# vccheng2001/DeepVCP-Pointcloud-Registration

Hardware: AMD Instinct MI355X
Metric: pairs/sec (full DeepVCP forward) at N=16384, K=64; rot/trans error vs ref (higher is better)
Workload: dtype f32

## Files before the change

### deepvcp-pointcloud-registration_amd/csrc/ball_query.hip

```cpp
#include "common.h"
#include "morton.h"


namespace dvcp {

template <typename T>
struct alignas(16) PointSS {
  T x, y, z, ss;
};

constexpr int kBqThreads = 256;

template <typename T>
__global__ __launch_bounds__(kBqThreads) void ball_query_kernel(
    PointsView<T> pts, int N, PointsView<T> ctr, int S, T r2, int nsample,
    int32_t* __restrict__ count, int32_t* __restrict__ list, int64_t* __restrict__ padded) {
  constexpr int TILE = (sizeof(T) == 4) ? 1024 : 512;
  __shared__ PointSS<T> tile[TILE];
  const int b = blockIdx.y;
  const int s = blockIdx.x * kBqThreads + threadIdx.x;
  const bool live = s < S;
  T cx = 0, cy = 0, cz = 0;
  if (live) {
    cx = ctr.at(b, 0, s);
    cy = ctr.at(b, 1, s);
    cz = ctr.at(b, 2, s);
  }
  const T ssc = sumsq3(cx, cy, cz);
  const int64_t row = (static_cast<int64_t>(b) * S + s) * nsample;
  int32_t* my_list = list ? list + row : nullptr;
  int64_t* my_pad = padded ? padded + row : nullptr;
  int cnt = 0;
  int first = N;
  bool done = !live;

  for (int t0 = 0; t0 < N; t0 += TILE) {
    const int nt = min(TILE, N - t0);
    __syncthreads();
    for (int j = threadIdx.x; j < nt; j += kBqThreads) {
      const T x = pts.at(b, 0, t0 + j), y = pts.at(b, 1, t0 + j), z = pts.at(b, 2, t0 + j);
      tile[j] = PointSS<T>{x, y, z, sumsq3(x, y, z)};
    }
    __syncthreads();
    if (!done) {
      for (int j = 0; j < nt; ++j) {
        const PointSS<T> p = tile[j];
        const T d2 = expansion_d2(dot3_blas(cx, cy, cz, p.x, p.y, p.z), ssc, p.ss);
        if (!(d2 > r2)) {
          const int n = t0 + j;
          if (cnt == 0) first = n;
          if (my_list) my_list[cnt] = n;
          if (my_pad) my_pad[cnt] = n;
          if (++cnt == nsample) {
            done = true;
            break;
          }
        }
      }
    }
    if (__syncthreads_and(done)) break;
  }
  if (!live) return;
  if (count) count[static_cast<int64_t>(b) * S + s] = cnt;
  if (my_list && cnt == 0) my_list[0] = 0;
  if (my_pad)
    for (int j = cnt; j < nsample; ++j) my_pad[j] = first;
}


__host__ __device__ constexpr int bq_padded_n(int N) { return (N + 15) & ~15; }

constexpr int kBqTile = 64;
#ifndef DVCP_BQ_ABL
#define DVCP_BQ_ABL 0
#endif
constexpr int kBqMaxTiles = 1024;
constexpr int kBqSmallTiles = 256;
constexpr int kBqCap = 256;

struct BqLayout {
  float4* packed;
  float4* sorted;
  float4* tbox;
  int32_t* cperm;
};

inline int64_t bq_align(int64_t x) { return (x + 255) & ~int64_t(255); }

inline BqLayout bq_layout(void* ws, int B, int N, int S) {
  const int64_t T = ceil_div(N, kBqTile);
  char* p = static_cast<char*>(ws);
  BqLayout L;
  L.packed = reinterpret_cast<float4*>(p);
  p += bq_align(16 * int64_t(B) * bq_padded_n(N));
  L.sorted = reinterpret_cast<float4*>(p);
  p += bq_align(16 * int64_t(B) * T * kBqTile);
  L.tbox = reinterpret_cast<float4*>(p);
  p += bq_align(32 * int64_t(B) * T);
  L.cperm = reinterpret_cast<int32_t*>(p);
  return L;
}

inline int64_t bq_workspace_bytes(int B, int N, int S) {
  const int64_t T = ceil_div(N, kBqTile);
  return bq_align(16 * int64_t(B) * bq_padded_n(N)) + bq_align(16 * int64_t(B) * T * kBqTile) +
         bq_align(32 * int64_t(B) * T) + bq_align(4 * int64_t(B) * S);
}

__global__ void bq_pack_kernel(PointsView<float> pts, int N, float4* __restrict__ packed) {
  const int b = blockIdx.y;
  const int n = blockIdx.x * blockDim.x + threadIdx.x;
  const int np = bq_padded_n(N);
  if (n >= np) return;
  float4 v = make_float4(0.f, 0.f, 0.f, 0.f);
  if (n < N) {
    const float x = pts.at(b, 0, n), y = pts.at(b, 1, n), z = pts.at(b, 2, n);
    v = make_float4(x, y, z, sumsq3(x, y, z));
  }
  packed[static_cast<int64_t>(b) * np + n] = v;
}

__global__ __launch_bounds__(kBuildThreads) void bq_build_kernel(PointsView<float> pts, int N, PointsView<float> ctr,
                                                                 int S, BqLayout L, int tiled) {
  __shared__ uint32_t bins[kSortBins];
  __shared__ uint32_t boxk[kBqMaxTiles][6];
  __shared__ uint32_t wsum[16];
  __shared__ float red[2][3][16];
  const int b = blockIdx.y, tid = threadIdx.x;
  auto get_ctr = [&](int i, float (&v)[3]) {
#pragma unroll
    for (int a = 0; a < 3; ++a) v[a] = ctr.at(b, a, i);
  };
  float lo[3], hi[3];
  if (blockIdx.x == 1) {
    block_bbox(S, get_ctr, lo, hi, red);
    int32_t* cp = L.cperm + static_cast<int64_t>(b) * S;
    morton_sort(
        S, get_ctr, [&](int pos, int i, const float (&)[3]) { cp[pos] = i; }, lo, hi, bins, wsum);
    return;
  }
  const int np = bq_padded_n(N);
  float4* pk = L.packed + static_cast<int64_t>(b) * np;
  for (int i = tid; i < np; i += kBuildThreads) {
    float4 v = make_float4(0.f, 0.f, 0.f, 0.f);
    if (i < N) {
      const float x = pts.at(b, 0, i), y = pts.at(b, 1, i), z = pts.at(b, 2, i);
      v = make_float4(x, y, z, sumsq3(x, y, z));
    }
    pk[i] = v;
  }
  if (!tiled) return;
  const int T = (N + kBqTile - 1) / kBqTile;
  float4* so = L.sorted + static_cast<int64_t>(b) * T * kBqTile;
  for (int i = tid; i < T * 6; i += kBuildThreads) boxk[i / 6][i % 6] = (i % 6) < 3 ? 0xFFFFFFFFu : 0u;
  auto get_pt = [&](int i, float (&v)[3]) {
#pragma unroll
    for (int a = 0; a < 3; ++a) v[a] = pts.at(b, a, i);
  };
  block_bbox(N, get_pt, lo, hi, red);
  morton_sort(
      N, get_pt,
      [&](int pos, int i, const float (&v)[3]) {
        so[pos] = make_float4(v[0], v[1], v[2], __int_as_float(i));
        const int t = pos / kBqTile;
        const bool fin = __builtin_isfinite(v[0]) && __builtin_isfinite(v[1]) && __builtin_isfinite(v[2]);
#pragma unroll
        for (int a = 0; a < 3; ++a) {
          atomicMin(&boxk[t][a], float_order(fin ? v[a] : -__builtin_huge_valf()));
          atomicMax(&boxk[t][3 + a], float_order(fin ? v[a] : __builtin_huge_valf()));
        }
      },
      lo, hi, bins, wsum);
  for (int pos = N + tid; pos < T * kBqTile; pos += kBuildThreads)
    so[pos] = make_float4(__builtin_nanf(""), __builtin_nanf(""), __builtin_nanf(""), __int_as_float(0x7FFFFFFF));
  for (int t = tid; t < T; t += kBuildThreads) {
    float4* tb = L.tbox + (static_cast<int64_t>(b) * T + t) * 2;
    tb[0] = make_float4(float_unorder(boxk[t][0]), float_unorder(boxk[t][1]), float_unorder(boxk[t][2]), 0.f);
    tb[1] = make_float4(float_unorder(boxk[t][3]), float_unorder(boxk[t][4]), float_unorder(boxk[t][5]), 0.f);
  }
}

__global__ __launch_bounds__(256) void bq_wave_kernel(const float4* __restrict__ packed, int N, PointsView<float> ctr,
                                                      int S, float r2, int nsample, int32_t* __restrict__ count,
                                                      int32_t* __restrict__ list, int64_t* __restrict__ padded) {
  const int b = blockIdx.y;
  const int s = blockIdx.x * 256 + threadIdx.x;
  if ((blockIdx.x * 256 + (threadIdx.x & ~63)) >= S) return;
  const bool live = s < S;
  float cx = 0.f, cy = 0.f, cz = 0.f;
  if (live) {
    cx = ctr.at(b, 0, s);
    cy = ctr.at(b, 1, s);
    cz = ctr.at(b, 2, s);
  }
  const float ssc = sumsq3(cx, cy, cz);
  const int64_t row = (static_cast<int64_t>(b) * S + s) * nsample;
  int cnt = live ? 0 : nsample;
  int first = N;
  const const_float* P = (const const_float*)uniform_ptr(packed + static_cast<int64_t>(b) * bq_padded_n(N));
  for (int n0 = 0; n0 < N; n0 += 16) {
    float c[64];
#pragma unroll
    for (int u = 0; u < 64; ++u) c[u] = P[4 * n0 + u];
#pragma unroll
    for (int j = 0; j < 16; ++j) {
      const int n = n0 + j;
      const float d2 = expansion_d2(dot3_blas(cx, cy, cz, c[4 * j], c[4 * j + 1], c[4 * j + 2]), ssc, c[4 * j + 3]);
      if ((n < N) & !(d2 > r2) & (cnt < nsample)) {
        first = cnt == 0 ? n : first;
        if (list) list[row + cnt] = n;
        if (padded) padded[row + cnt] = n;
        ++cnt;
      }
    }
    if (__ballot(cnt < nsample) == 0) break;
  }
  if (!live) return;
  if (count) count[static_cast<int64_t>(b) * S + s] = cnt;
  if (list && cnt == 0) list[row] = 0;
  if (padded)
    for (int j = cnt; j < nsample; ++j) padded[row + j] = first;
}

__device__ __forceinline__ float wave_fmin(float v) {
  for (int off = 32; off > 0; off >>= 1) v = fminf(v, __shfl_xor(v, off, kWave));
  return v;
}
__device__ __forceinline__ float wave_fmax(float v) {
  for (int off = 32; off > 0; off >>= 1) v = fmaxf(v, __shfl_xor(v, off, kWave));
  return v;
}

__device__ __forceinline__ float bq_prune_thr(float r2, float ssc_max, float ssp_max) {
  return (r2 + 0x1p-20f * (ssc_max + ssp_max)) * (1.0f + 0x1p-19f);
}

__device__ __forceinline__ float box_ss_max(float lx, float ly, float lz, float hx, float hy, float hz) {
  const float ax = fmaxf(fabsf(lx), fabsf(hx)), ay = fmaxf(fabsf(ly), fabsf(hy)), az = fmaxf(fabsf(lz), fabsf(hz));
  return ((ax * ax + ay * ay) + az * az) * (1.0f + 0x1p-20f);
}

__device__ __forceinline__ float bq_gap(float lo, float hi, float v_lo, float v_hi) {
  return fmaxf(fmaxf(v_lo - hi, lo - v_hi), 0.0f);
}

template <int MAXT>
__global__ __launch_bounds__(256) void bq_tiled_kernel(BqLayout L, int N, PointsView<float> ctr, int S, float r2,
                                                       int nsample, int32_t* __restrict__ count,
                                                       int32_t* __restrict__ list, int64_t* __restrict__ padded,
                                                       int xcd) {
  __shared__ uint32_t bm[4][MAXT * 2];
  __shared__ float4 cpt[4][kBqCap];
  __shared__ int32_t cid[4][kBqCap];
  int b = blockIdx.y, bx = blockIdx.x;
  if (xcd) {
    const int lin = static_cast<int>(blockIdx.y * gridDim.x + blockIdx.x);
    const int slot = lin >> 3;
    b = (lin & 7) + 8 * (slot / static_cast<int>(gridDim.x));
    bx = slot % static_cast<int>(gridDim.x);
  }
  const int wave = threadIdx.x >> 6, lane = threadIdx.x & 63;
  const int q0 = (bx * 4 + wave) * 64;
  if (q0 >= S) return;
  const int T = (N + kBqTile - 1) / kBqTile;
  const int NW = (N + 31) >> 5;
  const int np = bq_padded_n(N);
  const bool live = q0 + lane < S;
  const int s = live ? L.cperm[static_cast<int64_t>(b) * S + q0 + lane] : 0;
  float cx = 0.f, cy = 0.f, cz = 0.f;
  if (live) {
    cx = ctr.at(b, 0, s);
    cy = ctr.at(b, 1, s);
    cz = ctr.at(b, 2, s);
  }
  const float ssc = sumsq3(cx, cy, cz);
  const bool fin = __builtin_isfinite(cx) && __builtin_isfinite(cy) && __builtin_isfinite(cz);
  const float inf = __builtin_huge_valf();
  int cut1 = -1, cut2 = -1, cut3 = -1;
  if (__ballot(live && !fin) == 0) {
    const float rr2 = 2.0f * sqrtf(r2);
    const bool bl = live;
    auto box_vol = [&](const float (&lo)[3], const float (&hi)[3]) {
      return !(hi[0] >= lo[0]) ? 0.0f : ((hi[0] - lo[0] + rr2) * (hi[1] - lo[1] + rr2)) * (hi[2] - lo[2] + rr2);
    };
    auto best_cut = [&](int a, int e) -> int {
      const bool in = bl && lane >= a && lane < e;
      const float c3[3] = {cx, cy, cz};
      float plo[3], phi[3], slo[3], shi[3];
#pragma unroll
      for (int d = 0; d < 3; ++d) {
        plo[d] = slo[d] = in ? c3[d] : inf;
        phi[d] = shi[d] = in ? c3[d] : -inf;
      }
#pragma unroll
      for (int off = 1; off < 64; off <<= 1) {
#pragma unroll
        for (int d = 0; d < 3; ++d) {
          const float ul = __shfl_up(plo[d], off, kWave), uh = __shfl_up(phi[d], off, kWave);
          const float dl = __shfl_down(slo[d], off, kWave), dh = __shfl_down(shi[d], off, kWave);
          if (lane >= off) {
            plo[d] = fminf(plo[d], ul);
            phi[d] = fmaxf(phi[d], uh);
          }
          if (lane + off < 64) {
            slo[d] = fminf(slo[d], dl);
            shi[d] = fmaxf(shi[d], dh);
          }
        }
      }
      const float vp = box_vol(plo, phi);
      const float vs = box_vol(slo, shi);
      const float vprev = __shfl_up(vp, 1, kWave);
      const float whole = __shfl(vp, 63, kWave);
      const float cost = (lane > a && lane < e) ? vprev + vs : inf;
      float m = cost;
      for (int off = 32; off > 0; off >>= 1) m = fminf(m, __shfl_xor(m, off, kWave));
      if (!(m < 0.7f * whole)) return -1;
      return static_cast<int>(__builtin_ctzll(__ballot(cost == m)));
    };
    cut1 = best_cut(0, 64);
    if (cut1 > 0) {
      cut2 = best_cut(0, cut1);
      cut3 = best_cut(cut1, 64);
    }
  }
  const int ngroups = 1 + (cut1 >= 0) + (cut2 >= 0) + (cut3 >= 0);
  const int gid = (cut2 >= 0 && lane >= cut2) + (cut1 >= 0 && lane >= cut1) + (cut3 >= 0 && lane >= cut3);
  uint32_t* mybm = bm[wave];
  const float4* tb = L.tbox + static_cast<int64_t>(b) * T * 2;
  const float4* so = L.sorted + static_cast<int64_t>(b) * T * kBqTile;
  const float4* pk = L.packed + static_cast<int64_t>(b) * np;
  const int64_t row = (static_cast<int64_t>(b) * S + s) * nsample;
  int cnt = live ? 0 : nsample;
  int first = N;
  float4* mypt = cpt[wave];
  int32_t* myid = cid[wave];
  for (int g = 0; g < ngroups; ++g) {
    const bool act = live && gid == g;
    if (__ballot(act) == 0) continue;
    const float wlx = wave_fmin(act ? (fin ? cx : -inf) : inf), whx = wave_fmax(act ? (fin ? cx : inf) : -inf);
    const float wly = wave_fmin(act ? (fin ? cy : -inf) : inf), why = wave_fmax(act ? (fin ? cy : inf) : -inf);
    const float wlz = wave_fmin(act ? (fin ? cz : -inf) : inf), whz = wave_fmax(act ? (fin ? cz : inf) : -inf);
    const float ssc_max = wave_fmax(act && fin ? ssc : 0.0f);

    __builtin_amdgcn_fence(__ATOMIC_ACQ_REL, "wavefront");
    __builtin_amdgcn_wave_barrier();
    for (int i = lane; i < NW; i += 64) mybm[i] = 0u;
    __builtin_amdgcn_fence(__ATOMIC_RELEASE, "wavefront");
    __builtin_amdgcn_wave_barrier();
    for (int t0 = 0; t0 < T; t0 += 64) {
      const int t = t0 + lane;
      bool cand = false;
      if (t < T) {
        const float4 lo = tb[2 * t], hi = tb[2 * t + 1];
        const float gx = bq_gap(lo.x, hi.x, wlx, whx), gy = bq_gap(lo.y, hi.y, wly, why), gz = bq_gap(lo.z, hi.z, wlz, whz);
        const float lb2 = (gx * gx + gy * gy) + gz * gz;
        cand = !(lb2 > bq_prune_thr(r2, ssc_max, box_ss_max(lo.x, lo.y, lo.z, hi.x, hi.y, hi.z)));
      }
      uint64_t mask = __ballot(cand);
      while (mask) {
        int tt[4];
#pragma unroll
        for (int u = 0; u < 4; ++u) {
          tt[u] = mask ? t0 + __builtin_ctzll(mask) : -1;
          mask &= mask - 1;
        }
        float4 q[4];
#pragma unroll
        for (int u = 0; u < 4; ++u) q[u] = so[max(tt[u], 0) * kBqTile + lane];
#pragma unroll
        for (int u = 0; u < 4; ++u) {
          const int idx = __float_as_int(q[u].w);
          const float gx = bq_gap(q[u].x, q[u].x, wlx, whx), gy = bq_gap(q[u].y, q[u].y, wly, why),
                      gz = bq_gap(q[u].z, q[u].z, wlz, whz);
          const float lb2 = (gx * gx + gy * gy) + gz * gz;
          const float ssp = ((q[u].x * q[u].x + q[u].y * q[u].y) + q[u].z * q[u].z) * (1.0f + 0x1p-20f);
          if (tt[u] >= 0 && idx < N && !(lb2 > bq_prune_thr(r2, ssc_max, ssp)))
            atomicOr(&mybm[idx >> 5], 1u << (idx & 31));
        }
      }
    }
    __builtin_amdgcn_fence(__ATOMIC_ACQ_REL, "wavefront");
    __builtin_amdgcn_wave_barrier();

    for (int c0 = 0; c0 < NW; c0 += 64) {
      const uint32_t word = (c0 + lane < NW) ? mybm[c0 + lane] : 0u;
      const int pc = __builtin_popcount(word);
      int incl = pc;
#pragma unroll
      for (int off = 1; off < 64; off <<= 1) {
        const int u = __shfl_up(incl, off, kWave);
        if (lane >= off) incl += u;
      }
      const int total = __shfl(incl, 63, kWave);
      const int excl = incl - pc;
      for (int base = 0; base < total; base += kBqCap) {
        int p = excl;
        uint32_t wd = word;
        while (wd && p < base + kBqCap) {
          const int bit = __builtin_ctz(wd);
          wd &= wd - 1;
          if (p >= base) myid[p - base] = (c0 + lane) * 32 + bit;
          ++p;
        }
        __builtin_amdgcn_fence(__ATOMIC_ACQ_REL, "wavefront");
        __builtin_amdgcn_wave_barrier();
        const int nc = min(kBqCap, total - base);
#pragma unroll
        for (int u = 0; u < kBqCap / 64; ++u) {
          const int j = u * 64 + lane;
          if (j < nc) mypt[j] = pk[myid[j]];
        }
        __builtin_amdgcn_fence(__ATOMIC_ACQ_REL, "wavefront");
        __builtin_amdgcn_wave_barrier();
        for (int j0 = 0; j0 < nc; j0 += 64) {
          const int je = min(nc, j0 + 64);
          for (int j1 = j0; j1 < je; j1 += 8) {
            float4 q[8];
#pragma unroll
            for (int u = 0; u < 8; ++u) q[u] = mypt[j1 + u];
#pragma unroll
            for (int u = 0; u < 8; ++u) {
              const float d2 = expansion_d2(dot3_blas(cx, cy, cz, q[u].x, q[u].y, q[u].z), ssc, q[u].w);
              if (act & (j1 + u < je) & !(d2 > r2) & (cnt < nsample)) {
                const int n = myid[j1 + u];
                first = cnt == 0 ? n : first;
#if DVCP_BQ_ABL != 1
                if (list) list[row + cnt] = n;
#endif
                if (padded) padded[row + cnt] = n;
                ++cnt;
              }
            }
          }
          if (__ballot(act && cnt < nsample) == 0) goto group_done;
        }
        __builtin_amdgcn_fence(__ATOMIC_ACQ_REL, "wavefront");
        __builtin_amdgcn_wave_barrier();
      }
    }
  group_done:;
  }
  if (!live) return;
  if (count) count[static_cast<int64_t>(b) * S + s] = cnt;
  if (list && cnt == 0) list[row] = 0;
  if (padded)
    for (int j = cnt; j < nsample; ++j) padded[row + j] = first;
}

template <typename T>
__global__ void square_distance_kernel(PointsView<T> src, int S, PointsView<T> dst, int N, T* __restrict__ out) {
  const int b = blockIdx.z;
  const int s = blockIdx.y;
  const int n = blockIdx.x * blockDim.x + threadIdx.x;
  if (n >= N) return;
  const T sx = src.at(b, 0, s), sy = src.at(b, 1, s), sz = src.at(b, 2, s);
  const T dx = dst.at(b, 0, n), dy = dst.at(b, 1, n), dz = dst.at(b, 2, n);
  out[(static_cast<int64_t>(b) * S + s) * N + n] =
      expansion_d2(dot3_blas(sx, sy, sz, dx, dy, dz), sumsq3(sx, sy, sz), sumsq3(dx, dy, dz));
}

template <typename T>
static int launch_bq(const void* xyz, int64_t sb, int64_t sc, int64_t sn, int N, const void* c, int64_t cb,
                     int64_t cc, int64_t cn, int S, int B, double radius, int nsample, int32_t* count,
                     int32_t* list, int64_t* padded, void* workspace, hipStream_t st) {
  PointsView<T> pv{static_cast<const T*>(xyz), sb, sc, sn};
  PointsView<T> cv{static_cast<const T*>(c), cb, cc, cn};
  const T r2 = static_cast<T>(radius * radius);
  if constexpr (sizeof(T) == 4) {
    if (workspace) {
      const BqLayout L = bq_layout(workspace, B, N, S);
      const int tiled = N <= kBqMaxTiles * kBqTile;
      hipLaunchKernelGGL(bq_build_kernel, dim3(tiled ? 2 : 1, B), dim3(kBuildThreads), 0, st, pv, N, cv, S, L, tiled);
      if (int e = launch_status("dvcp_ball_query(build)")) return e;
      if (tiled)
        hipLaunchKernelGGL(N <= kBqSmallTiles * kBqTile ? bq_tiled_kernel<kBqSmallTiles> : bq_tiled_kernel<kBqMaxTiles>,
                           dim3(ceil_div(S, 256), B), dim3(256), 0, st, L, N, cv, S, r2, nsample, count, list, padded,
                           B % 8 == 0 ? 1 : 0);
      else
        hipLaunchKernelGGL(bq_wave_kernel, dim3(ceil_div(S, 256), B), dim3(256), 0, st, L.packed, N, cv, S, r2,
                           nsample, count, list, padded);
      return launch_status("dvcp_ball_query");
    }
  }
  dim3 grid(ceil_div(S, kBqThreads), B);
  hipLaunchKernelGGL((ball_query_kernel<T>), grid, dim3(kBqThreads), 0, st, pv, N, cv, S, r2, nsample, count,
                     list, padded);
  return launch_status("dvcp_ball_query");
}

}

extern "C" int dvcp_ball_query_ws(int dtype, const void* xyz, int64_t sb, int64_t sc, int64_t sn, int N,
                                  const void* ctr, int64_t cb, int64_t cc, int64_t cn, int S, int B,
                                  double radius, int nsample, int32_t* count, int32_t* list,
                                  int64_t* padded, void* workspace, void* stream) {
  DVCP_REQUIRE(xyz && ctr, "dvcp_ball_query: null pointer");
  DVCP_REQUIRE(N >= 0 && S >= 0 && B >= 0 && nsample > 0, "dvcp_ball_query: bad sizes");
  if (B == 0 || S == 0) return DVCP_OK;
  DVCP_REQUIRE(B <= 65535, "dvcp_ball_query: B too large");
  hipStream_t st = static_cast<hipStream_t>(stream);
  if (dtype == DVCP_F32)
    return dvcp::launch_bq<float>(xyz, sb, sc, sn, N, ctr, cb, cc, cn, S, B, radius, nsample, count, list,
                                  padded, workspace, st);
  if (dtype == DVCP_F64)
    return dvcp::launch_bq<double>(xyz, sb, sc, sn, N, ctr, cb, cc, cn, S, B, radius, nsample, count, list,
                                   padded, nullptr, st);
  dvcp::set_error("dvcp_ball_query: bad dtype %d", dtype);
  return DVCP_EINVAL;
}

extern "C" int64_t dvcp_ball_query_workspace_bytes(int B, int N, int S) {
  if (B < 0 || N < 0 || S < 0) return -1;
  return dvcp::bq_workspace_bytes(B, N, S);
}

extern "C" int dvcp_ball_query(int dtype, const void* xyz, int64_t sb, int64_t sc, int64_t sn, int N,
                               const void* ctr, int64_t cb, int64_t cc, int64_t cn, int S, int B,
                               double radius, int nsample, int32_t* count, int32_t* list,
                               int64_t* padded, void* stream) {
  return dvcp_ball_query_ws(dtype, xyz, sb, sc, sn, N, ctr, cb, cc, cn, S, B, radius, nsample, count, list, padded,
                            nullptr, stream);
}

extern "C" int dvcp_square_distance(int dtype, const void* src, int64_t sb, int64_t sc, int64_t sn, int S,
                                    const void* dst, int64_t db, int64_t dc, int64_t dn, int N, int B,
                                    void* out, void* stream) {
  DVCP_REQUIRE(src && dst && out, "dvcp_square_distance: null pointer");
  if (B == 0 || S == 0 || N == 0) return DVCP_OK;
  DVCP_REQUIRE(S <= 65535 && B <= 65535, "dvcp_square_distance: S/B too large");
  hipStream_t st = static_cast<hipStream_t>(stream);
  dim3 grid(dvcp::ceil_div(N, 256), S, B);
  if (dtype == DVCP_F32) {
    hipLaunchKernelGGL((dvcp::square_distance_kernel<float>), grid, dim3(256), 0, st,
                       dvcp::PointsView<float>{static_cast<const float*>(src), sb, sc, sn}, S,
                       dvcp::PointsView<float>{static_cast<const float*>(dst), db, dc, dn}, N,
                       static_cast<float*>(out));
  } else if (dtype == DVCP_F64) {
    hipLaunchKernelGGL((dvcp::square_distance_kernel<double>), grid, dim3(256), 0, st,
                       dvcp::PointsView<double>{static_cast<const double*>(src), sb, sc, sn}, S,
                       dvcp::PointsView<double>{static_cast<const double*>(dst), db, dc, dn}, N,
                       static_cast<double*>(out));
  } else {
    dvcp::set_error("dvcp_square_distance: bad dtype %d", dtype);
    return DVCP_EINVAL;
  }
  return dvcp::launch_status("dvcp_square_distance");
}
```

Before: 2531.

## Assign four lanes per query center in tiled ball query kernel

Restructures the tiled ball-query kernel so each wavefront handles 16 centers with 4 lanes per center. Candidates are split across the quad and hits are compacted in order with a ballot-based prefix. The candidate-bitmap compaction now walks contiguous per-lane word ranges instead of strided words. Group splitting drops from up to four groups to a single cut, candidate ids are stored as uint16, and launch bounds gain an occupancy hint. The aim is more parallelism per query and less serial hit scanning, at the cost of four times as many blocks, repeated tile culling per wave, and uint16 ids that limit indexable N.

```diff
diff --git a/deepvcp-pointcloud-registration_amd/csrc/ball_query.hip b/deepvcp-pointcloud-registration_amd/csrc/ball_query.hip
--- a/deepvcp-pointcloud-registration_amd/csrc/ball_query.hip
+++ b/deepvcp-pointcloud-registration_amd/csrc/ball_query.hip
@@ -71,12 +71,11 @@
 __host__ __device__ constexpr int bq_padded_n(int N) { return (N + 15) & ~15; }
 
 constexpr int kBqTile = 64;
-#ifndef DVCP_BQ_ABL
-#define DVCP_BQ_ABL 0
-#endif
 constexpr int kBqMaxTiles = 1024;
 constexpr int kBqSmallTiles = 256;
 constexpr int kBqCap = 256;
+constexpr int kBqQuad = 4;
+constexpr int kBqWaveCtr = kWave / kBqQuad;
 
 struct BqLayout {
   float4* packed;
@@ -230,6 +229,9 @@
   for (int off = 32; off > 0; off >>= 1) v = fmaxf(v, __shfl_xor(v, off, kWave));
   return v;
 }
+__device__ __forceinline__ float wave_uniform(float v) {
+  return __int_as_float(__builtin_amdgcn_readfirstlane(__float_as_int(v)));
+}
 
 __device__ __forceinline__ float bq_prune_thr(float r2, float ssc_max, float ssp_max) {
   return (r2 + 0x1p-20f * (ssc_max + ssp_max)) * (1.0f + 0x1p-19f);
@@ -245,13 +247,13 @@
 }
 
 template <int MAXT>
-__global__ __launch_bounds__(256) void bq_tiled_kernel(BqLayout L, int N, PointsView<float> ctr, int S, float r2,
-                                                       int nsample, int32_t* __restrict__ count,
-                                                       int32_t* __restrict__ list, int64_t* __restrict__ padded,
-                                                       int xcd) {
-  __shared__ uint32_t bm[4][MAXT * 2];
+__global__ __launch_bounds__(256, MAXT == kBqSmallTiles ? 6 : 3) void bq_tiled_kernel(
+    BqLayout L, int N, PointsView<float> ctr, int S, float r2, int nsample, int32_t* __restrict__ count,
+    int32_t* __restrict__ list, int64_t* __restrict__ padded, int xcd) {
+  constexpr int WPL = MAXT * 2 / kWave;
+  __shared__ alignas(16) uint32_t bm[4][MAXT * 2];
   __shared__ float4 cpt[4][kBqCap];
-  __shared__ int32_t cid[4][kBqCap];
+  __shared__ uint16_t cid[4][kBqCap];
   int b = blockIdx.y, bx = blockIdx.x;
   if (xcd) {
     const int lin = static_cast<int>(blockIdx.y * gridDim.x + blockIdx.x);
@@ -260,13 +262,13 @@
     bx = slot % static_cast<int>(gridDim.x);
   }
   const int wave = threadIdx.x >> 6, lane = threadIdx.x & 63;
-  const int q0 = (bx * 4 + wave) * 64;
+  const int ctrl = lane / kBqQuad, ql = lane % kBqQuad;
+  const int q0 = (bx * 4 + wave) * kBqWaveCtr;
   if (q0 >= S) return;
   const int T = (N + kBqTile - 1) / kBqTile;
-  const int NW = (N + 31) >> 5;
   const int np = bq_padded_n(N);
-  const bool live = q0 + lane < S;
-  const int s = live ? L.cperm[static_cast<int64_t>(b) * S + q0 + lane] : 0;
+  const bool live = q0 + ctrl < S;
+  const int s = live ? L.cperm[static_cast<int64_t>(b) * S + q0 + ctrl] : 0;
   float cx = 0.f, cy = 0.f, cz = 0.f;
   if (live) {
     cx = ctr.at(b, 0, s);
@@ -276,56 +278,57 @@
   const float ssc = sumsq3(cx, cy, cz);
   const bool fin = __builtin_isfinite(cx) && __builtin_isfinite(cy) && __builtin_isfinite(cz);
   const float inf = __builtin_huge_valf();
-  int cut1 = -1, cut2 = -1, cut3 = -1;
+  int cut = -1;
   if (__ballot(live && !fin) == 0) {
     const float rr2 = 2.0f * sqrtf(r2);
-    const bool bl = live;
     auto box_vol = [&](const float (&lo)[3], const float (&hi)[3]) {
       return !(hi[0] >= lo[0]) ? 0.0f : ((hi[0] - lo[0] + rr2) * (hi[1] - lo[1] + rr2)) * (hi[2] - lo[2] + rr2);
     };
-    auto best_cut = [&](int a, int e) -> int {
-      const bool in = bl && lane >= a && lane < e;
-      const float c3[3] = {cx, cy, cz};
-      float plo[3], phi[3], slo[3], shi[3];
+    const float c3[3] = {cx, cy, cz};
+    float lo[3], hi[3];
+#pragma unroll
+    for (int d = 0; d < 3; ++d) {
+      lo[d] = live ? c3[d] : inf;
+      hi[d] = live ? c3[d] : -inf;
+    }
+#pragma unroll
+    for (int off = kBqQuad; off < kWave; off <<= 1) {
 #pragma unroll
       for (int d = 0; d < 3; ++d) {
-        plo[d] = slo[d] = in ? c3[d] : inf;
-        phi[d] = shi[d] = in ? c3[d] : -inf;
-      }
-#pragma unroll
-      for (int off = 1; off < 64; off <<= 1) {
-#pragma unroll
-        for (int d = 0; d < 3; ++d) {
-          const float ul = __shfl_up(plo[d], off, kWave), uh = __shfl_up(phi[d], off, kWave);
-          const float dl = __shfl_down(slo[d], off, kWave), dh = __shfl_down(shi[d], off, kWave);
-          if (lane >= off) {
-            plo[d] = fminf(plo[d], ul);
-            phi[d] = fmaxf(phi[d], uh);
-          }
-          if (lane + off < 64) {
-            slo[d] = fminf(slo[d], dl);
-            shi[d] = fmaxf(shi[d], dh);
-          }
-        }
-      }
-      const float vp = box_vol(plo, phi);
-      const float vs = box_vol(slo, shi);
-      const float vprev = __shfl_up(vp, 1, kWave);
-      const float whole = __shfl(vp, 63, kWave);
-      const float cost = (lane > a && lane < e) ? vprev + vs : inf;
-      float m = cost;
-      for (int off = 32; off > 0; off >>= 1) m = fminf(m, __shfl_xor(m, off, kWave));
-      if (!(m < 0.7f * whole)) return -1;
-      return static_cast<int>(__builtin_ctzll(__ballot(cost == m)));
-    };
-    cut1 = best_cut(0, 64);
-    if (cut1 > 0) {
-      cut2 = best_cut(0, cut1);
-      cut3 = best_cut(cut1, 64);
-    }
-  }
-  const int ngroups = 1 + (cut1 >= 0) + (cut2 >= 0) + (cut3 >= 0);
-  const int gid = (cut2 >= 0 && lane >= cut2) + (cut1 >= 0 && lane >= cut1) + (cut3 >= 0 && lane >= cut3);
+        const float ul = __shfl_up(lo[d], off, kWave), uh = __shfl_up(hi[d], off, kWave);
+        if (lane >= off) {
+          lo[d] = fminf(lo[d], ul);
+          hi[d] = fmaxf(hi[d], uh);
+        }
+      }
+    }
+    const float vp = box_vol(lo, hi);
+#pragma unroll
+    for (int d = 0; d < 3; ++d) {
+      lo[d] = live ? c3[d] : inf;
+      hi[d] = live ? c3[d] : -inf;
+    }
+#pragma unroll
+    for (int off = kBqQuad; off < kWave; off <<= 1) {
+#pragma unroll
+      for (int d = 0; d < 3; ++d) {
+        const float dl = __shfl_down(lo[d], off, kWave), dh = __shfl_down(hi[d], off, kWave);
+        if (lane + off < kWave) {
+          lo[d] = fminf(lo[d], dl);
+          hi[d] = fmaxf(hi[d], dh);
+        }
+      }
+    }
+    const float vs = box_vol(lo, hi);
+    const float vprev = __shfl_up(vp, kBqQuad, kWave);
+    const float whole = __shfl(vp, kWave - 1, kWave);
+    const float cost = ctrl > 0 ? vprev + vs : inf;
+    float m = cost;
+    for (int off = 32; off > 0; off >>= 1) m = fminf(m, __shfl_xor(m, off, kWave));
+    if (m < 0.7f * whole) cut = static_cast<int>(__builtin_ctzll(__ballot(cost == m))) / kBqQuad;
+  }
+  const int ngroups = 1 + (cut >= 0);
+  const int gid = cut >= 0 && ctrl >= cut;
   uint32_t* mybm = bm[wave];
   const float4* tb = L.tbox + static_cast<int64_t>(b) * T * 2;
   const float4* so = L.sorted + static_cast<int64_t>(b) * T * kBqTile;
@@ -334,18 +337,22 @@
   int cnt = live ? 0 : nsample;
   int first = N;
   float4* mypt = cpt[wave];
-  int32_t* myid = cid[wave];
+  uint16_t* myid = cid[wave];
   for (int g = 0; g < ngroups; ++g) {
     const bool act = live && gid == g;
     if (__ballot(act) == 0) continue;
-    const float wlx = wave_fmin(act ? (fin ? cx : -inf) : inf), whx = wave_fmax(act ? (fin ? cx : inf) : -inf);
-    const float wly = wave_fmin(act ? (fin ? cy : -inf) : inf), why = wave_fmax(act ? (fin ? cy : inf) : -inf);
-    const float wlz = wave_fmin(act ? (fin ? cz : -inf) : inf), whz = wave_fmax(act ? (fin ? cz : inf) : -inf);
-    const float ssc_max = wave_fmax(act && fin ? ssc : 0.0f);
+    const float wlx = wave_uniform(wave_fmin(act ? (fin ? cx : -inf) : inf)),
+                whx = wave_uniform(wave_fmax(act ? (fin ? cx : inf) : -inf));
+    const float wly = wave_uniform(wave_fmin(act ? (fin ? cy : -inf) : inf)),
+                why = wave_uniform(wave_fmax(act ? (fin ? cy : inf) : -inf));
+    const float wlz = wave_uniform(wave_fmin(act ? (fin ? cz : -inf) : inf)),
+                whz = wave_uniform(wave_fmax(act ? (fin ? cz : inf) : -inf));
+    const float ssc_max = wave_uniform(wave_fmax(act && fin ? ssc : 0.0f));
 
     __builtin_amdgcn_fence(__ATOMIC_ACQ_REL, "wavefront");
     __builtin_amdgcn_wave_barrier();
-    for (int i = lane; i < NW; i += 64) mybm[i] = 0u;
+#pragma unroll
+    for (int k = 0; k < WPL; ++k) mybm[k * kWave + lane] = 0u;
     __builtin_amdgcn_fence(__ATOMIC_RELEASE, "wavefront");
     __builtin_amdgcn_wave_barrier();
     for (int t0 = 0; t0 < T; t0 += 64) {
@@ -383,69 +390,79 @@
     __builtin_amdgcn_fence(__ATOMIC_ACQ_REL, "wavefront");
     __builtin_amdgcn_wave_barrier();
 
-    for (int c0 = 0; c0 < NW; c0 += 64) {
-      const uint32_t word = (c0 + lane < NW) ? mybm[c0 + lane] : 0u;
-      const int pc = __builtin_popcount(word);
-      int incl = pc;
-#pragma unroll
-      for (int off = 1; off < 64; off <<= 1) {
-        const int u = __shfl_up(incl, off, kWave);
-        if (lane >= off) incl += u;
-      }
-      const int total = __shfl(incl, 63, kWave);
-      const int excl = incl - pc;
-      for (int base = 0; base < total; base += kBqCap) {
-        int p = excl;
-        uint32_t wd = word;
-        while (wd && p < base + kBqCap) {
-          const int bit = __builtin_ctz(wd);
-          wd &= wd - 1;
-          if (p >= base) myid[p - base] = (c0 + lane) * 32 + bit;
-          ++p;
-        }
-        __builtin_amdgcn_fence(__ATOMIC_ACQ_REL, "wavefront");
-        __builtin_amdgcn_wave_barrier();
-        const int nc = min(kBqCap, total - base);
-#pragma unroll
-        for (int u = 0; u < kBqCap / 64; ++u) {
-          const int j = u * 64 + lane;
-          if (j < nc) mypt[j] = pk[myid[j]];
-        }
-        __builtin_amdgcn_fence(__ATOMIC_ACQ_REL, "wavefront");
-        __builtin_amdgcn_wave_barrier();
-        for (int j0 = 0; j0 < nc; j0 += 64) {
-          const int je = min(nc, j0 + 64);
-          for (int j1 = j0; j1 < je; j1 += 8) {
-            float4 q[8];
-#pragma unroll
-            for (int u = 0; u < 8; ++u) q[u] = mypt[j1 + u];
-#pragma unroll
-            for (int u = 0; u < 8; ++u) {
-              const float d2 = expansion_d2(dot3_blas(cx, cy, cz, q[u].x, q[u].y, q[u].z), ssc, q[u].w);
-              if (act & (j1 + u < je) & !(d2 > r2) & (cnt < nsample)) {
-                const int n = myid[j1 + u];
-                first = cnt == 0 ? n : first;
-#if DVCP_BQ_ABL != 1
-                if (list) list[row + cnt] = n;
-#endif
-                if (padded) padded[row + cnt] = n;
-                ++cnt;
-              }
-            }
+    const uint4* myw4 = reinterpret_cast<const uint4*>(mybm + lane * WPL);
+    int pc = 0;
+#pragma unroll
+    for (int k = 0; k < WPL / 4; ++k) {
+      const uint4 w = myw4[k];
+      pc += (__builtin_popcount(w.x) + __builtin_popcount(w.y)) + (__builtin_popcount(w.z) + __builtin_popcount(w.w));
+    }
+    int incl = pc;
+#pragma unroll
+    for (int off = 1; off < kWave; off <<= 1) {
+      const int u = __shfl_up(incl, off, kWave);
+      if (lane >= off) incl += u;
+    }
+    const int total = __shfl(incl, kWave - 1, kWave);
+    int p = incl - pc;
+    int wk = lane * WPL;
+    uint32_t wd = 0u;
+    for (int base = 0; base < total; base += kBqCap) {
+      const int pend = min(base + kBqCap, incl);
+      while (p < pend) {
+        if (wd == 0u) {
+          wd = mybm[wk++];
+          continue;
+        }
+        myid[p - base] = static_cast<uint16_t>((wk - 1) * 32 + __builtin_ctz(wd));
+        wd &= wd - 1;
+        ++p;
+      }
+      __builtin_amdgcn_fence(__ATOMIC_ACQ_REL, "wavefront");
+      __builtin_amdgcn_wave_barrier();
+      const int nc = min(kBqCap, total - base);
+#pragma unroll
+      for (int u = 0; u < kBqCap / kWave; ++u) {
+        const int j = u * kWave + lane;
+        if (j < nc) mypt[j] = pk[myid[j]];
+      }
+      __builtin_amdgcn_fence(__ATOMIC_ACQ_REL, "wavefront");
+      __builtin_amdgcn_wave_barrier();
+      for (int j0 = 0; j0 < nc; j0 += 4 * kBqQuad) {
+        float4 q[4];
+#pragma unroll
+        for (int u = 0; u < 4; ++u) q[u] = mypt[j0 + u * kBqQuad + ql];
+#pragma unroll
+        for (int u = 0; u < 4; ++u) {
+          const int j = j0 + u * kBqQuad + ql;
+          const float d2 = expansion_d2(dot3_blas(cx, cy, cz, q[u].x, q[u].y, q[u].z), ssc, q[u].w);
+          const bool hit = act & (j < nc) & !(d2 > r2) & (cnt < nsample);
+          const uint32_t qb = static_cast<uint32_t>(__ballot(hit) >> (lane - ql)) & ((1u << kBqQuad) - 1u);
+          const int slot = cnt + __builtin_popcount(qb & ((1u << ql) - 1u));
+          if (hit && slot < nsample) {
+            const int n = myid[j];
+            if (slot == 0) first = n;
+            if (list) list[row + slot] = n;
+            if (padded) padded[row + slot] = n;
           }
-          if (__ballot(act && cnt < nsample) == 0) goto group_done;
-        }
-        __builtin_amdgcn_fence(__ATOMIC_ACQ_REL, "wavefront");
-        __builtin_amdgcn_wave_barrier();
-      }
+          cnt = min(cnt + __builtin_popcount(qb), nsample);
+        }
+        if (__ballot(act && cnt < nsample) == 0) goto group_done;
+      }
+      __builtin_amdgcn_fence(__ATOMIC_ACQ_REL, "wavefront");
+      __builtin_amdgcn_wave_barrier();
     }
   group_done:;
   }
+  first = min(first, __shfl_xor(first, 1, kWave));
+  first = min(first, __shfl_xor(first, 2, kWave));
   if (!live) return;
-  if (count) count[static_cast<int64_t>(b) * S + s] = cnt;
-  if (list && cnt == 0) list[row] = 0;
+  if (ql == 0) {
+    if (count) count[static_cast<int64_t>(b) * S + s] = cnt;
+    if (list && cnt == 0) list[row] = 0;
+  }
   if (padded)
-    for (int j = cnt; j < nsample; ++j) padded[row + j] = first;
+    for (int j = cnt + ql; j < nsample; j += kBqQuad) padded[row + j] = first;
 }
 
 template <typename T>
@@ -475,8 +492,8 @@
       if (int e = launch_status("dvcp_ball_query(build)")) return e;
       if (tiled)
         hipLaunchKernelGGL(N <= kBqSmallTiles * kBqTile ? bq_tiled_kernel<kBqSmallTiles> : bq_tiled_kernel<kBqMaxTiles>,
-                           dim3(ceil_div(S, 256), B), dim3(256), 0, st, L, N, cv, S, r2, nsample, count, list, padded,
-                           B % 8 == 0 ? 1 : 0);
+                           dim3(ceil_div(S, 4 * kBqWaveCtr), B), dim3(256), 0, st, L, N, cv, S, r2, nsample, count, list,
+                           padded, B % 8 == 0 ? 1 : 0);
       else
         hipLaunchKernelGGL(bq_wave_kernel, dim3(ceil_div(S, 256), B), dim3(256), 0, st, L.packed, N, cv, S, r2,
                            nsample, count, list, padded);
```

Result: no change. 2526 (-0.2%).
